# rpp0/gr-lora

Hardware: AMD Instinct MI355X
Metric: IQ Msamples/s demodulated (higher is better)
Workload: dtype f32

## Files before the change

gr_lora_amd/capi.py:

```python
from __future__ import annotations

import ctypes as C
import os
from typing import List, Optional, Sequence, Tuple

import numpy as np

_HERE = os.path.dirname(os.path.abspath(__file__))
LIB_PATH = os.environ.get("LORA_HIP_LIB") or os.path.join(_HERE, "liblora_hip.so")

DEMOD_GRAD, DEMOD_FFT, DEMOD_FFT_COMPAT = 0, 1, 2
FLAG_TRACE = 1
FLAG_PIN_HOST = 2
FLAG_FAST_SYNC = 4
FLAG_NO_DECOUPLED = 8
IQ_CF32, IQ_SC16, IQ_SC8, IQ_CU8 = 0, 1, 2, 3

EXPORTS = [
    "lora_hip_abi_version", "lora_hip_strerror", "lora_hip_last_error", "lora_hip_create", "lora_hip_destroy",
    "lora_hip_get_geometry", "lora_hip_set_sf", "lora_hip_set_samp_rate", "lora_hip_work", "lora_hip_flush",
    "lora_hip_decode_device", "lora_hip_frames_available", "lora_hip_poll_frame", "lora_hip_drain_frames", "lora_hip_drain_slots", "lora_hip_demod_symbols_device", "lora_hip_demod_symbols_ex_device",
    "lora_hip_last_timing", "lora_hip_last_plan", "lora_hip_get_table", "lora_hip_last_payload_pass", "lora_hip_gap_starts_device", "lora_hip_decode_device_begin", "lora_hip_decode_device_end", "lora_hip_decode_device_prepass", "lora_hip_trace", "lora_hip_trace_clear", "lora_hip_check_frame", "lora_hip_estimate_cfo_device", "lora_hip_ref_ifreq_device",
    "lora_hip_set_stream_latency", "lora_hip_stream_info", "lora_hip_walker_kernel_name", "lora_hip_window_stats_device", "lora_hip_detect_preambles_device", "lora_hip_decode_at_headers_device",
    "lora_hip_mux_create", "lora_hip_mux_destroy", "lora_hip_mux_work", "lora_hip_mux_flush", "lora_hip_mux_set_latency", "lora_hip_mux_set_max_ahead", "lora_hip_mux_frames_available",
    "lora_hip_mux_poll_frame", "lora_hip_mux_passes", "lora_hip_mux_last_error",
    "lora_hip_iq_item_bytes", "lora_hip_iq_unpack_device", "lora_hip_work_raw",
]


EXPORTS_CHANNELIZER = [
    "lora_hip_channelizer_create", "lora_hip_channelizer_destroy", "lora_hip_channelizer_last_error", "lora_hip_channelizer_taps",
    "lora_hip_channelizer_output_items", "lora_hip_channelizer_run_device", "lora_hip_channelizer_work", "lora_hip_channelizer_apply_cfo",
    "lora_hip_channelizer_last_kernel_ms", "lora_hip_channelizer_run_device_raw", "lora_hip_channelizer_work_raw",
]


EXPORTS_FILTERBANK = [
# ... 144 lines not shown
    L.lora_hip_get_geometry.argtypes = [vp, C.POINTER(C.c_uint32), C.POINTER(C.c_uint32), C.POINTER(C.c_uint32)]
    L.lora_hip_set_sf.argtypes = [vp, C.c_uint8]
    L.lora_hip_set_samp_rate.argtypes = [vp, C.c_float]
    L.lora_hip_work.argtypes = [vp, vp, C.c_size_t, C.POINTER(C.c_size_t)]
    L.lora_hip_flush.argtypes = [vp]
    L.lora_hip_decode_device.argtypes = [vp, vp, C.c_size_t, vp, vp, C.c_uint32, vp]
    L.lora_hip_frames_available.restype = C.c_size_t
    L.lora_hip_frames_available.argtypes = [vp]
    L.lora_hip_poll_frame.argtypes = [vp, vp, C.c_size_t, C.POINTER(C.c_size_t), C.POINTER(FrameInfo)]
    L.lora_hip_drain_frames.argtypes = [vp, vp, C.c_size_t, C.POINTER(FrameInfo), C.c_size_t, C.POINTER(C.c_size_t)]
    L.lora_hip_drain_slots.argtypes = [vp, vp, C.c_size_t, C.c_size_t, C.POINTER(C.c_size_t)]
    L.lora_hip_demod_symbols_device.argtypes = [vp, vp, C.c_size_t, vp, C.c_size_t, C.c_int, vp, vp]
    L.lora_hip_demod_symbols_ex_device.argtypes = [vp, vp, C.c_size_t, vp, C.c_size_t, C.c_int, vp, vp, vp]
    L.lora_hip_last_timing.argtypes = [vp, C.POINTER(Timing)]
    L.lora_hip_last_plan.argtypes = [vp, C.POINTER(C.c_uint32), C.POINTER(C.c_uint32)]
    L.lora_hip_last_payload_pass.argtypes = [vp, C.POINTER(C.c_uint32), C.POINTER(C.c_uint32), C.POINTER(C.c_uint32), C.POINTER(C.c_uint32), C.POINTER(C.c_uint32), C.POINTER(C.c_float)]
    L.lora_hip_decode_device_begin.argtypes = [vp, vp, C.c_size_t, vp, vp, C.c_uint32, vp, C.c_uint32]
    L.lora_hip_decode_device_end.argtypes = [vp]
    L.lora_hip_decode_device_prepass.argtypes = [vp, vp, C.c_size_t, vp, vp, C.c_uint32, vp, C.c_uint32]
    L.lora_hip_gap_starts_device.argtypes = [vp, vp, C.c_size_t, vp, vp, C.c_uint32, vp, C.c_size_t, vp, vp]
    L.lora_hip_trace.restype = C.c_size_t
    L.lora_hip_trace.argtypes = [vp, C.POINTER(C.POINTER(Step))]
    L.lora_hip_trace_clear.argtypes = [vp]
    L.lora_hip_trace_clear.restype = None
    L.lora_hip_estimate_cfo_device.argtypes = [vp, vp, C.c_size_t, C.POINTER(C.c_int64), C.c_size_t, C.c_int, C.POINTER(C.c_float), vp]
    L.lora_hip_estimate_cfo_device.restype = C.c_int
    L.lora_hip_ref_ifreq_device.argtypes = [vp, vp, C.c_size_t, C.POINTER(C.c_float), C.POINTER(C.c_float), vp]
    L.lora_hip_ref_ifreq_device.restype = C.c_int
    if hasattr(L, "lora_hip_get_table") or not os.environ.get("LORA_HIP_LIB"):
        L.lora_hip_get_table.argtypes = [vp, C.c_int, C.POINTER(C.c_float), C.c_size_t, C.POINTER(C.c_size_t)]
# ... 325 lines not shown
        self._check(self.L.lora_hip_last_plan(self.h, C.byref(b), C.byref(n)))
        return bool(b.value), int(n.value)

    def table(self, which: int) -> np.ndarray:
        n = C.c_size_t()
        self._check(self.L.lora_hip_get_table(self.h, which, None, 0, C.byref(n)))
        out = np.empty(n.value, np.float32)
        self._check(self.L.lora_hip_get_table(self.h, which, out.ctypes.data_as(C.POINTER(C.c_float)), n.value, C.byref(n)))
        return out

    def payload_pass(self):
        a, mv, b, r, c, m = C.c_uint32(0), C.c_uint32(0), C.c_uint32(0), C.c_uint32(0), C.c_uint32(0), C.c_float(0)
        self._check(self.L.lora_hip_last_payload_pass(self.h, C.byref(a), C.byref(mv), C.byref(b), C.byref(r), C.byref(c), C.byref(m)))
        return dict(packets=int(a.value), moved=int(mv.value), rerun=int(b.value), rounds=int(r.value), symbols=int(c.value), ms=float(m.value))

    def trace(self):
        p = C.POINTER(Step)()
        n = self.L.lora_hip_trace(self.h, C.byref(p))
        return [(p[i].state, p[i].pos, p[i].consumed, p[i].bin, p[i].fine, p[i].value, p[i].stream, p[i].cycles) for i in range(n)]

    def trace_clear(self):
        self.L.lora_hip_trace_clear(self.h)


class Mux:

    def __init__(self, n_channels, samp_rate=1e6, bandwidth=125000, sf=7, implicit=False, cr=4, crc=True, reduced_rate=False,
                 disable_drift_correction=False, device=0, demod=DEMOD_FFT_COMPAT, flags=0, segment_symbols=0, batch_items=0):
        self.L = load()
        cfg = Config(struct_size=C.sizeof(Config), samp_rate=float(samp_rate), bandwidth=int(bandwidth), sf=int(sf), implicit=int(bool(implicit)), cr=int(cr),
# ... 366 lines not shown
```

gr_lora_amd/csrc/lora_device.h:

```cpp
#pragma once
#include <stdint.h>

#if !defined(__HIPCC__) && !defined(HIP_INCLUDE_HIP_HIP_RUNTIME_H)
struct float2 { float x, y; };
#endif

namespace lora_hip {

constexpr int kWG = 256;
constexpr int kMaxBinsPerThread = 16;
constexpr int kMaxFrame = 3 + 255 + 2;
constexpr int kMaxCodewords = 640;

enum DecState : int32_t { kDetect = 0, kSync, kFindSfd, kPause, kDecodeHeader, kDecodePayload, kStop };

enum AttemptStatus : uint32_t {
    kAttemptNone = 0,
    kAttemptFrame = 1,
    kAttemptLostSync = 2,
    kAttemptOutOfData = 3,
    kAttemptAtHeader = 4,
    kAttemptAtSfd = 5,
    kAttemptHeaderOnly = 6
};
// ... 73 lines not shown
    int64_t  final_pos;
    uint32_t n_attempts;
    uint32_t final_cr;
    uint32_t npush;
    float    push_tail[4];
    uint32_t stop_reason;
    uint32_t n_steps;
    uint32_t pad;
    uint32_t cyc[6];
    uint32_t rounds[6];
    int64_t  tail_final_pos;
    uint32_t tail_valid, tail_first_rec, tail_n_attempts, tail_final_cr, tail_npush, tail_stop_reason, tail_pad, tail_rsv;
    float    tail_push_tail[4];
    uint32_t ctl[4];
    uint32_t dbg[6];
};

struct StepRec {
    int32_t  state, consumed;
    int64_t  pos;
    int32_t  bin, fine;
    float    value;
    uint32_t stream;
    uint32_t cycles;
    uint32_t pad;
};

struct LaunchCfg {
    const float2 *iq;
    const Job *jobs;
    JobResult *results;
    AttemptRec *recs;
    uint32_t recs_per_job;
    float *scratch;
    StepRec *trace;
    uint32_t trace_cap;
    uint32_t n_jobs;
    uint32_t *balance;
    uint32_t skip_payload;
};
constexpr uint32_t kBalanceCus = 2048;
constexpr uint32_t kBalanceWords = 3u * kBalanceCus;

struct EnvStream {
    uint64_t off;
    uint32_t first_block;
    uint32_t n_blocks;
};
int launch_envelope(const float2 *iq, const EnvStream *streams , uint32_t n_streams, uint32_t sps,
                    float *d_E, unsigned long long *d_bitmap , void *stream);

int launch_walker(const DevParams &p, const LaunchCfg &c, void *stream);
const char *walker_kernel_name(const DevParams &p);
struct DemodAlt { int32_t *shift; uint32_t *bins; int32_t *fine; int64_t max_start; };
// ... 23 lines not shown
bool walker_has_skip_variant(const DevParams &p);
int launch_ref_ifreq(const float2 *x, uint32_t n, float *d_arg, float *d_ifreq, void *stream);
int launch_cfo(const DevParams &p, const float2 *iq, const int64_t *d_offsets, uint32_t n, int mode, float *d_out, void *stream);
bool walker3_covers(uint32_t sf);
uint32_t w3_tw_entries(uint32_t sf);
void build_w3_tables(uint32_t sf, float2 *tw, float2 *ctab );
uint32_t wave_tables_floats(uint32_t sf);
void build_wave_tables(uint32_t sf, const float2 *down, float *out);
uint32_t wave_tables_floats_d(uint32_t sf, uint32_t decim);
void build_wave_tables_d(uint32_t sf, uint32_t decim, const float2 *down, float *out);
uint32_t team_tables_entries(uint32_t sf);
void build_team_tables(uint32_t sf, const float2 *down, double dt, double bandwidth, float2 *out);
uint32_t walker_lds_bytes(const DevParams &p);
uint32_t walker_resident_slots(const DevParams &p);
uint32_t walker_resident_slots_full(const DevParams &p);
const char *walker_kernel_name_for(const DevParams &p, uint32_t n_jobs, bool skip = false);

}
```

gr_lora_amd/csrc/lora_kernels.hip:

```cpp

#include <hip/hip_runtime.h>
#include <math.h>
#include <stdio.h>
#include <atomic>
#include <cstdlib>
#include <stdint.h>
#include <type_traits>

#include "lora_device.h"
#include "whitening_data.inc"

namespace lora_hip {

__constant__ unsigned char c_whiten_cr56[LORA_WHITEN_CR56_LEN];
__constant__ unsigned char c_whiten_cr78[LORA_WHITEN_CR78_LEN];
__constant__ unsigned char c_h84_decode[256];
static std::atomic<bool> g_consts_ready[16];

static unsigned char h_hamming_encode(unsigned v)
{
    const unsigned b0 = v & 1u, b1 = (v >> 1) & 1u, b2 = (v >> 2) & 1u, b3 = (v >> 3) & 1u;
    const unsigned p1 = b1 ^ b2 ^ b3, p2 = b0 ^ b1 ^ b2, p3 = b0 ^ b1 ^ b3, p4 = b0 ^ b2 ^ b3;
    return (unsigned char)(p1 | (b0 << 1) | (b1 << 2) | (b2 << 3) | (p2 << 4) | (b3 << 5) | (p3 << 6) | (p4 << 7));
}
// ... 1053 lines not shown
            cus_dev = dev;
        }
        if (n_jobs <= (uint32_t)cus && !no_wide) {
            const bool grad = p.demod_mode == 0u;
            if (p.sf == 8u && !grad) { k.fn = walker2_kernel_sf8_wide; k.name = "walker2_kernel_sf8_wide"; }
            else if (p.sf == 7u && !grad) { k.fn = walker2_kernel_sf7_wide; k.name = "walker2_kernel_sf7_wide"; }
            else if (p.sf == 7u) { k.fn = walker2_kernel_sf7_grad_wide; k.name = "walker2_kernel_sf7_grad_wide"; }
            else { k.fn = walker2_kernel_sf8_grad_wide; k.name = "walker2_kernel_sf8_grad_wide"; }
        }
    }
    return k;
}

const char *walker_kernel_name_for(const DevParams &p, uint32_t n_jobs, bool skip) { return pick_for_launch(p, n_jobs, skip).name; }

int launch_walker(const DevParams &p, const LaunchCfg &c, void *stream)
{
    if (ensure_constants() != 0) return -1;
    if (c.skip_payload && !walker_has_skip_variant(p)) return -1;
    const WalkerKernel k = pick_for_launch(p, c.n_jobs, c.skip_payload != 0);
    if (k.lds > 64u * 1024u) {
        static thread_local const void *last_fn = nullptr;
        static thread_local uint32_t last_lds = 0;
        static thread_local int last_dev = -1;
        int dev = 0;
        (void)hipGetDevice(&dev);
        if (last_fn != (const void *)k.fn || last_lds < k.lds || last_dev != dev) {
            if (hipFuncSetAttribute((const void *)k.fn, hipFuncAttributeMaxDynamicSharedMemorySize, (int)k.lds) != hipSuccess) return -1;
            last_fn = (const void *)k.fn; last_lds = k.lds; last_dev = dev;
        }
// ... 255 lines not shown
```

gr_lora_amd/csrc/lora_runtime.cpp:

```cpp

#include <hip/hip_runtime.h>

#include <algorithm>
#include <cmath>
#include <cstddef>
#include <cstdarg>
#include <cstdio>
#include <cstdlib>
#include <cstring>
#include <chrono>
#include <deque>
#include <new>
#include <string>
#include <vector>

#include "../../include/lora_hip.h"
#include "lora_device.h"
#include "lora_stitch.hpp"
#include "lora_mux_dev.h"
#include "lora_iq.h"

using namespace lora_hip;

namespace {
// ... 101 lines not shown
    DevBuf<Job> d_jobs;
    DevBuf<JobResult> d_results;
    DevBuf<AttemptRec> d_recs;
    DevBuf<float> d_scratch;
    DevBuf<StepRec> d_trace;
    DevBuf<float2> d_staging;
    DevBuf<int64_t> d_offsets;
    DevBuf<uint32_t> d_bins;
    RunOut run_out[2];
    std::vector<JobResult> h_results;
    std::vector<AttemptRec> h_recs;
    std::vector<StepRec> h_trace;
    hipEvent_t ev0 = nullptr, ev1 = nullptr, ev_done = nullptr;
    hipEvent_t ev_pre0 = nullptr, ev_pre1 = nullptr, ev_dep = nullptr;
    hipStream_t pre_stream = nullptr;
    struct Pending { uint32_t nj = 0, recs_per_job = 0, eager = 0, trace_cap = 0; bool direct = true, open = false; hipStream_t st = nullptr;
                     std::chrono::steady_clock::time_point hp0, hp1; } pending;
    PassCtx pass;
    std::vector<StreamDesc> pass_streams;
    const float2 *pass_iq = nullptr;
    hipStream_t pass_st = nullptr;
    bool pass_open = false, iq_ready = false;
    bool pre_issued = false;
    const float2 *pre_iq = nullptr;
    uint64_t pre_sig = 0;
    uint32_t pre_ns = 0;
    std::chrono::steady_clock::time_point pre_hq0;
    FrameQueue frames;
    PinnedBuf<Job> p_jobs;
    PinnedBuf<JobResult> p_res;
    PinnedBuf<AttemptRec> p_recs;
// ... 9 lines not shown
    ChunkPipe pipe;
    struct HostFeed {
        PinnedBuf<float2> stage[2];
        hipEvent_t stage_ev[2] = {nullptr, nullptr};
        bool stage_busy[2] = {false, false};
        int stage_i = 0;
        DevBuf<uint32_t> d_raw;
        std::vector<std::pair<uintptr_t, uintptr_t>> pinned;
        std::vector<std::pair<uintptr_t, uintptr_t>> refused;
    } feed;
    const char *last_kernel = nullptr;
    uint32_t last_kernel_jobs = 0;
    uint32_t resident_slots = 0;
    uint32_t resident_slots_alt = ~0u;
    uint32_t eager_recs = 4;
    uint32_t last_plan_burst = 0, last_plan_segments = 0;
    int decoupled_policy = -1;
    bool launch_skip = false;
    uint32_t dec_backoff = 0;
    uint32_t last_payload_packets = 0, last_payload_rerun = 0, last_payload_symbols = 0, last_payload_moved = 0, last_payload_rounds = 0;
    float last_payload_ms = 0.0f;
    PinnedBuf<int64_t> p_pay_off;
    PinnedBuf<PayloadDesc> p_pay_desc;
    PinnedBuf<PayloadOut> p_pay_out;
    DevBuf<int32_t> d_fine, d_alt_shift, d_alt_fine;
    DevBuf<uint32_t> d_alt_bins;
    hipStream_t pay_stream = nullptr;
    hipEvent_t ev_pay0 = nullptr, ev_pay1 = nullptr, ev_pay_done = nullptr;
    struct PayState { std::vector<uint32_t> active; size_t used = 0, cap_sym = 0, n_sym = 0; int round = 0; float ms = 0.0f; bool open = false; } pay;
};
// ... 224 lines not shown
    HIP_TRY(h, h->p_recs.reserve((size_t)nj * eager));
    std::memcpy(h->p_jobs.p, jobs.data(), nj * sizeof(Job));
    if (!direct) HIP_TRY(h, hipMemcpyAsync(h->d_jobs.p, h->p_jobs.p, nj * sizeof(Job), hipMemcpyHostToDevice, st));
    LaunchCfg c{};
    c.iq = d_iq; c.recs_per_job = recs_per_job;
    c.jobs = direct ? h->p_jobs.p : h->d_jobs.p; c.results = direct ? h->p_res.p : h->d_results.p; c.recs = direct ? h->p_recs.p : h->d_recs.p;
    c.scratch = need_scratch ? h->d_scratch.p : nullptr;
    c.trace = trace_cap ? h->d_trace.p : nullptr; c.trace_cap = trace_cap; c.n_jobs = nj;
    static const bool no_balance = getenv("LORA_HIP_NO_BALANCE") != nullptr;
    if (!h->d_balance.p && !no_balance) {
        HIP_TRY(h, h->d_balance.reserve(kBalanceWords));
        HIP_TRY(h, hipMemsetAsync(h->d_balance.p, 0, kBalanceWords * sizeof(uint32_t), st));
    }
    c.balance = no_balance ? nullptr : h->d_balance.p;
    c.skip_payload = h->launch_skip ? 1u : 0u;
    HIP_TRY(h, hipEventRecord(h->ev0, st));
    if (nj >= h->last_kernel_jobs) { h->last_kernel = walker_kernel_name_for(h->P, nj, h->launch_skip); h->last_kernel_jobs = nj; }
    if (launch_walker(h->P, c, st) != 0) return fail(h, LORA_HIP_ERR_HIP, "walker launch failed: %s", hipGetErrorString(hipGetLastError()));
    HIP_TRY(h, hipEventRecord(h->ev1, st));
    if (!direct) {
        HIP_TRY(h, hipMemcpyAsync(h->p_res.p, h->d_results.p, nj * sizeof(JobResult), hipMemcpyDeviceToHost, st));
        HIP_TRY(h, hipMemcpy2DAsync(h->p_recs.p, eager * sizeof(AttemptRec), h->d_recs.p, recs_per_job * sizeof(AttemptRec), eager * sizeof(AttemptRec), nj,
                                    hipMemcpyDeviceToHost, st));
    }
    HIP_TRY(h, hipEventRecord(h->ev_done, st));
    h->pending.eager = eager; h->pending.direct = direct; h->pending.open = true;
    h->pending.hp1 = std::chrono::steady_clock::now();
    return LORA_HIP_OK;
}

// ... 61 lines not shown
    }
    if (dbg_stats && h->P.use_fast) {
        double sync_rounds = 0; uint32_t frames = 0, tails = 0, early = 0;
        for (uint32_t j = 0; j < nj; j++) {
            const JobResult &r = out.res[j];
            sync_rounds += r.rounds[1];
            const uint32_t used = std::min(std::min(eager, max_att), r.n_attempts + (r.tail_valid ? r.tail_n_attempts : 0u));
            for (uint32_t a = 0; a < used; a++) {
                const AttemptRec &t = out.recs[(size_t)j * stride + a];
                frames += (a < r.n_attempts && t.status == kAttemptFrame) ? 1u : 0u;
                if (r.tail_valid && a + 1u == r.n_attempts + r.tail_n_attempts && r.tail_pad) { tails++; early += t.status == kAttemptAtSfd ? 1u : 0u; }
            }
        }
        fprintf(stderr, "[lora_hip] acquisitions: %.0f SYNC rounds for %u frames of this launch (%.2f per frame); %u tail probes reached a packet, %u of them stopped behind their first FIND_SFD step\n",
                sync_rounds, frames, frames ? sync_rounds / frames : 0.0, tails, early);
    }
    h->eager_recs = std::min(std::max(max_att, 2u), 8u);
    bool more = false;
    if (max_att > eager) {
        HIP_TRY(h, hipMemcpy2DAsync(out.recs.data() + eager, stride * sizeof(AttemptRec), h->d_recs.p + eager,
                                    recs_per_job * sizeof(AttemptRec), (max_att - eager) * sizeof(AttemptRec), nj, hipMemcpyDeviceToHost, st));
        more = true;
    }
    if (trace_cap) {
        h->h_trace.resize((size_t)nj * trace_cap);
        HIP_TRY(h, hipMemcpyAsync(h->h_trace.data(), h->d_trace.p, (size_t)nj * trace_cap * sizeof(StepRec), hipMemcpyDeviceToHost, st));
        more = true;
    }
    if (more) HIP_TRY(h, hipStreamSynchronize(st));
    float ms = 0.0f;
// ... 1373 lines not shown
    return LORA_HIP_OK;
}

lora_hip_status lora_hip_last_payload_pass(const lora_hip_decoder_t *h, uint32_t *packets, uint32_t *moved, uint32_t *rerun, uint32_t *rounds, uint32_t *symbols, float *ms)
{
    if (!h) return LORA_HIP_ERR_ARG;
    if (packets) *packets = h->last_payload_packets;
    if (moved) *moved = h->last_payload_moved;
    if (rounds) *rounds = h->last_payload_rounds;
    if (rerun) *rerun = h->last_payload_rerun;
    if (symbols) *symbols = h->last_payload_symbols;
    if (ms) *ms = h->last_payload_ms;
    return LORA_HIP_OK;
}

const char *lora_hip_walker_kernel_name(const lora_hip_decoder_t *h) { return h ? (h->last_kernel ? h->last_kernel : walker_kernel_name(h->P)) : ""; }

lora_hip_status lora_hip_last_timing(const lora_hip_decoder_t *h, lora_hip_timing_t *t)
{
    if (!h || !t) return LORA_HIP_ERR_ARG;
    *t = h->timing;
    return LORA_HIP_OK;
}

size_t lora_hip_trace(const lora_hip_decoder_t *h, const lora_hip_step_t **steps)
{
    if (!h || !steps) return 0;
    *steps = h->trace.data();
    return h->trace.size();
}
// ... 8 lines not shown
```

gr_lora_amd/csrc/lora_walker2.inc.hip:

```cpp

constexpr int kW2DetectK = 4;
#ifndef LORA_W2_WAVES_SF7
#define LORA_W2_WAVES_SF7 8
#endif
#ifndef LORA_W2_WAVES_SF8
#define LORA_W2_WAVES_SF8 8
#endif
#ifndef LORA_W2_SFD_K
#define LORA_W2_SFD_K 2
#endif
#ifndef LORA_W2_EU_SF8
#define LORA_W2_EU_SF8 4
#endif
constexpr int kW2MaxWaves = LORA_W2_WAVES_SF7 > LORA_W2_WAVES_SF8 ? LORA_W2_WAVES_SF7 : LORA_W2_WAVES_SF8;

constexpr int kW2SfdK = LORA_W2_SFD_K;

enum W2Mode : int32_t { kPlanExit = 0, kPlanDetect, kPlanSync, kPlanSfd, kPlanPause, kPlanDecode, kPlanFinalize };

struct alignas(16) W2Plan {
    int64_t pos;
    int32_t mode;
    int32_t buf;
    int32_t resolve_prev;
    int32_t n_win;
    int32_t prev_n;
    int32_t zmode;
};

struct alignas(16) W2State {
    int64_t  pos, att_start, att_trig, att_hdr;
// ... 21 lines not shown
    float    specf[kW2MaxWaves][4];
    float    detf[kW2MaxWaves * kW2DetectK][4];
    int32_t  detn[kW2MaxWaves];
    int32_t  speci[2][kW2MaxWaves][4];
    W2Plan   plan[2];
    Shared   sh;
    W2State  st;
    W2Stats  stats;
    int64_t  ph_start;
    uint32_t ph_go, ph_cr, ph_natt, ph_pad;
    uint32_t det_streak;
    uint32_t prio;
    uint32_t words_pk[2];
    strict::Cands sc;
    uint32_t words_pk16[4];
};

struct W2Tabs {
    const float  *v;
    const float  *dd;
    float        *scratch;
};

template <int WAVES>
__device__ __forceinline__ void w2_block_argmax_first(float &v, int &idx, float *red)
{
    const int lane = threadIdx.x & 63, wave = threadIdx.x >> 6;
#pragma unroll
    for (int o = 32; o > 0; o >>= 1) {
        const float ov = __shfl_xor(v, o, 64);
// ... 120 lines not shown
            S.state = kDecodePayload;
        }
        return false;
    }
    if (block_done && !P.implicit) S.payload_symbols -= (int32_t)(4u + S.cr);
    if (S.payload_symbols <= 0) {
        uint32_t n_bytes;
        if (S.cr >= 3u) n_bytes = (uint32_t)ceilf((float)S.n_cw * 4.0f / (4.0f + (float)S.cr));
        else n_bytes = (S.n_cw + 1u) / 2u;
        if (n_bytes > (uint32_t)(kMaxCodewords / 2 + 8)) n_bytes = kMaxCodewords / 2 + 8;
        S.fin_n_bytes = n_bytes;
        S.fin_plen = S.payload_length > 257u ? 257u : S.payload_length;
        return true;
    }
    return false;
}

template <int SF>
__device__ __forceinline__ float4 w2_detect_window(const float2 *p_)
{
    const auto p = (const __attribute__((address_space(1))) v2f *)p_;
    constexpr int SPS = 8 << SF, J = SPS / 64;
    const int lane = threadIdx.x & 63;
    float a0 = 0.f, a1 = 0.f, a2 = 0.f, a3 = 0.f;
    constexpr int B = J < 16 ? J : 16;
#pragma unroll
    for (int jb = 0; jb < J; jb += B) {
        v2f u[B], w[B];
#pragma unroll
        for (int j = 0; j < B; j++) u[j] = p[(jb + j) * 64 + lane];
// ... 312 lines not shown
        default:
            pl.mode = kPlanDecode; pl.n_win = kW2Win;
            if (S.state == kDecodePayload && !P.implicit) {
                const int32_t rem = S.payload_symbols - (int32_t)S.n_words;
                pl.n_win = rem < kW2Win ? (rem > 0 ? rem : 1) : kW2Win;
            }
            break;
        }
    };
    auto plan_from_state = [&](W2Plan &pl) { plan_from(S, pl); };

    W2Tabs T{vl, ddl, W.red};
    uint32_t *bal_mine = nullptr, *bal_other = nullptr;
    uint32_t bal_rem = 0xffffffffu, bal_seen = 0u, bal_slot = 0u;
    if (t0) W.prio = 0u;
    if (t0 && C.balance) {
        const uint32_t hw = __builtin_amdgcn_s_getreg((31 << 11) | 4), xcc = __builtin_amdgcn_s_getreg((31 << 11) | 20);
        const uint32_t cu = ((xcc & 7u) << 8) | ((hw >> 8) & 0xffu);
        bal_slot = atomicAdd(&C.balance[2u * kBalanceCus + cu], 1u) & 1u;
        bal_mine = C.balance + 2u * cu + bal_slot;
        bal_other = C.balance + 2u * cu + (bal_slot ^ 1u);
    }
    for (int phase = 0; phase < 2; phase++) {
    if (t0) {
        S = W2State{};
        S.state = kDetect; S.pos = job.start; S.cr = job.cr_prev; S.has_crc = P.ctor_crc;
        S.phdr[1] = (uint8_t)((P.ctor_cr << 5) | (P.ctor_crc << 4));
        S.att_start = job.start; S.att_trig = -1; S.att_hdr = -1; S.att_cr_prev = job.cr_prev;
        if (job.start_at_header && phase == 0) { S.state = kDecodeHeader; S.in_attempt = 1; S.att_trig = job.start; S.att_hdr = job.start; }
        if (phase == 0) W.stats = W2Stats{};
// ... 23 lines not shown
        if (t0 && bal_mine) {
            W.prio = (bal_rem > bal_seen || (bal_rem == bal_seen && bal_slot != 0u)) ? 1u : 0u;
            const int64_t target = phase == 0 ? job.scan_limit + (job.probe_limit > job.scan_limit ? 12 * (int64_t)sps : 0) : pos + 6 * (int64_t)sps;
            const int64_t left = (target - pos) / (int64_t)sps;
            bal_rem = left < 1 ? 1u : (left > 0x3fffffff ? 0x3fffffffu : (uint32_t)left);
            __hip_atomic_store(bal_mine, bal_rem, __ATOMIC_RELAXED, __HIP_MEMORY_SCOPE_AGENT);
            bal_seen = __hip_atomic_load(bal_other, __ATOMIC_RELAXED, __HIP_MEMORY_SCOPE_AGENT);
        }
        if (!is_ctl) {
            if (W.prio) __builtin_amdgcn_s_setprio(1); else __builtin_amdgcn_s_setprio(0);
        }
        const int64_t wpos = pos + (int64_t)wave * sps;

        if (plan_mode == kPlanDetect) {
            const int kd = plan_n_win;
            if (!is_ctl) {
                const int64_t dpos = pos + (int64_t)wave * kd * sps;
                int nvalid = 0;
                if (dpos + 2 * (int64_t)sps <= n_items) {
                    const int64_t fit = (n_items - dpos) / (int64_t)sps - 1;
                    nvalid = fit < kd ? (int)fit : kd;
                }
                float a[kW2DetectK][4];
                if (nvalid > 0) {
                    if (kd == 1) { const float4 r = w2_detect_window<GSF>(X + dpos); a[0][0] = r.x; a[0][1] = r.y; a[0][2] = r.z; a[0][3] = r.w; }
                    else w2_detect_windows<GSF, kW2DetectK>(X + dpos, nvalid, a);
                }
                if (lane == 0) {
                    W.detn[wave] = nvalid;
                    for (int i = 0; i < kW2DetectK; i++)
                        if (i < nvalid) { float *o = W.detf[wave * kW2DetectK + i]; o[0] = a[i][0]; o[1] = a[i][1]; o[2] = a[i][2]; o[3] = a[i][3]; }
// ... 9 lines not shown
                const bool valid = q < NW && qi < W.detn[qw];
                float autocorr = 0.0f, pushed = 0.0f, e2 = 0.0f;
                if (valid) {
                    const float *o = W.detf[qw * kW2DetectK + qi];
                    const float d0 = o[0], d1 = o[1], e1 = o[2];
                    e2 = o[3];
                    pushed = e1 / (float)sps;
                    const float sq = sqrtf(e1 * e2);
                    autocorr = hypotf(d0 / sq, d1 / sq);
                }
                const unsigned long long vmask = __ballot(valid), tmask = __ballot(valid && autocorr >= 0.90f);
                W.red[q] = pushed; W.red[64 + q] = e2; W.red[128 + q] = autocorr;
                __builtin_amdgcn_wave_barrier();
                if (t0) {
                    W2State L = S;
                    int64_t n_lim = (job.scan_limit - L.pos + (int64_t)sps - 1) / (int64_t)sps;
                    if (n_lim < 1) n_lim = 1;
                    const int n_valid = (~vmask == 0ull) ? 64 : __builtin_ctzll(~vmask);
                    int n_max = n_valid < NW ? n_valid : NW;
                    if ((int64_t)n_max > n_lim) n_max = (int)n_lim;
                    const int qt = tmask ? __builtin_ctzll(tmask) : 64;
                    const bool trig = qt < n_max;
                    const int nd = trig ? qt + 1 : n_max;
                    if (nd > 0) {
                        if (trace) {
                            for (int i = 0; i < nd; i++) {
                                if (L.n_steps + (uint32_t)i < C.trace_cap) {
                                    StepRec &r = trace[L.n_steps + (uint32_t)i];
                                    r.state = kDetect; r.consumed = (trig && i == nd - 1) ? 0 : (int32_t)sps; r.pos = L.pos + (int64_t)i * sps; r.bin = -1; r.fine = 0;
                                    r.value = W.red[128 + i]; r.stream = job.stream_id; r.cycles = (uint32_t)(clock64() - t_start); r.pad = 0;
// ... 152 lines not shown
        }

        if (plan_mode == kPlanFinalize) {
            const uint32_t n_cw = S.n_cw, cr = S.cr, n_bytes = S.fin_n_bytes, plen = S.fin_plen;
            decode_payload_bytes(sh, n_cw, cr, n_bytes);
            AttemptRec &r = recs[S.n_att];
            for (uint32_t i = threadIdx.x; i < plen; i += kW2) r.frame[3u + i] = (i < n_bytes) ? sh.dec[i] : 0;
            __syncthreads();
            if (t0) {
                r.frame[0] = S.phdr[0]; r.frame[1] = S.phdr[1]; r.frame[2] = S.phdr[2];
                r.frame_len = 3u + plen;
                S.frame_ok = 1;
                S.state = kDetect;
                S.n_words = 0; S.n_cw = 0;
                S.fin_pending = 0;
                w2_end_step(S, job, C, recs, trace, S.fin_st, S.fin_consumed, S.fin_bin, S.fin_fine, 0.0f, t_start);
                plan_from_state(next);
            }
            continue;
        }

        int64_t dpos = pos;
        int32_t dn = plan_n_win;
        if (plan_resolve_prev && plan_prev_n > 0) {
            const int rb = plan_buf ^ 1;
            const int32_t s_l = lane < plan_prev_n ? W.speci[rb][lane][0] : -1, f_l = lane < plan_prev_n ? W.speci[rb][lane][1] : 0;
            const unsigned long long moved = __ballot(s_l >= 0 && f_l != 0);
            if (moved) {
                const int wq = __builtin_ctzll(moved);
                const int32_t redo = plan_prev_n - (wq + 1);
// ... 95 lines not shown
            } else {
                plan_from(L, np, zreq);
            }
            const long long tr3 = clock64();
            if (t0) {
                next = np;
                S = L;
                if constexpr (W16) { W.words_pk16[0] = wpk[0]; W.words_pk16[1] = wpk[1]; W.words_pk16[2] = wpk[2]; W.words_pk16[3] = wpk[3]; }
                else { W.words_pk[0] = wpk[0]; W.words_pk[1] = wpk[1]; }
                asm volatile("s_waitcnt lgkmcnt(0)" ::: "memory");
                W.stats.ctl[0] += (uint32_t)((tr1 - tr0) >> 6); W.stats.ctl[1] += (uint32_t)((tr2 - tr1) >> 6); W.stats.ctl[2] += (uint32_t)((tr3 - tr2) >> 6);
                W.stats.ctl[3] += (uint32_t)((clock64() - tr3) >> 6);
                W.stats.cyc[4] += (uint32_t)((clock64() - tr0) >> 6); W.stats.rounds[4]++;
            }
        }
    }

    __syncthreads();
    if (t0) {
        const bool in_attempt = S.in_attempt != 0;
        if (in_attempt && S.n_att < rec_cap) {
            AttemptRec &r = recs[S.n_att];
            r.status = (S.stop_reason == 3) ? kAttemptAtHeader : kAttemptOutOfData;
            r.start_pos = S.att_start; r.trig_pos = S.att_trig; r.hdr_pos = S.att_hdr; r.end_pos = S.pos;
            r.npush = S.npush;
            for (int i = 0; i < 4; i++) r.push_tail[i] = S.push_tail[i];
            r.cr_prev = S.att_cr_prev; r.hdr_ambig = S.att_ambig; r.n_symbols = S.n_sym; r.frame_len = 0; r.n_sfd = 0;
        }
        JobResult &jr = C.results[jid];
        const int64_t e_pos = in_attempt ? S.att_start : S.pos;
// ... 10 lines not shown
            jr.pad = e_pad;
            jr.tail_valid = 0;
            go = job.probe_limit > job.scan_limit && S.stop_reason == 0 && !in_attempt && !trace && e_natt < C.recs_per_job;
            W.ph_go = go ? 1u : 0u; W.ph_start = e_pos; W.ph_cr = S.cr; W.ph_natt = e_natt; W.ph_pad = 0;
        } else {
            jr.tail_valid = 1; jr.tail_first_rec = W.ph_natt;
            jr.tail_final_pos = e_pos; jr.tail_n_attempts = e_natt; jr.tail_final_cr = S.cr; jr.tail_npush = e_npush;
            for (int i = 0; i < 4; i++) jr.tail_push_tail[i] = S.push_tail[i];
            jr.tail_stop_reason = (uint32_t)S.stop_reason; jr.tail_pad = e_pad; jr.tail_rsv = 0;
        }
        if (!go) {
            W2Stats &Q = W.stats;
            if (Q.prev_state >= 0) { Q.cyc[Q.prev_state] += (uint32_t)((clock64() - Q.prev_t) >> 6); Q.rounds[Q.prev_state]++; }
            for (int i = 0; i < 6; i++) { jr.cyc[i] = Q.cyc[i]; jr.rounds[i] = Q.rounds[i]; }
            for (int i = 0; i < 4; i++) jr.ctl[i] = Q.ctl[i];
            jr.dbg[0] = __builtin_amdgcn_s_getreg((31 << 11) | 4); jr.dbg[1] = __builtin_amdgcn_s_getreg((31 << 11) | 20);
            jr.dbg[2] = dbg_t0; jr.dbg[3] = (uint32_t)__builtin_amdgcn_s_memrealtime();
            jr.dbg[4] = dbg_c0; jr.dbg[5] = (uint32_t)(clock64() >> 6);
        }
    }
    if (phase == 1) break;
    __syncthreads();
    if (!W.ph_go) break;
    bal_rem = 0xffffffffu;
    {
        const int64_t st = W.ph_start;
        const uint32_t lo = __builtin_amdgcn_readfirstlane((uint32_t)st), hi = __builtin_amdgcn_readfirstlane((uint32_t)((uint64_t)st >> 32));
        const uint32_t natt = __builtin_amdgcn_readfirstlane(W.ph_natt);
        job.start = (int64_t)(((uint64_t)hi << 32) | lo);
        job.cr_prev = __builtin_amdgcn_readfirstlane(W.ph_cr);
// ... 58 lines not shown
```

include/lora_hip.h:

```cpp
#ifndef LORA_HIP_H
#define LORA_HIP_H

#include <stddef.h>
#include <stdint.h>

#ifdef __cplusplus
extern "C" {
#endif

#define LORA_HIP_ABI_VERSION 4

typedef enum lora_hip_status {
    LORA_HIP_OK = 0,
    LORA_HIP_ERR_BAD_SF = -1,
    LORA_HIP_ERR_BAD_CONFIG = -2,
    LORA_HIP_ERR_NO_DEVICE = -3,
    LORA_HIP_ERR_HIP = -4,
    LORA_HIP_ERR_NOMEM = -5,
    LORA_HIP_ERR_ARG = -6,
    LORA_HIP_ERR_OVERFLOW = -7,
    LORA_HIP_ERR_INTERNAL = -8
} lora_hip_status;

typedef enum lora_hip_iq_format {
// ... 133 lines not shown
                                      size_t max_frames, size_t *n_frames);

lora_hip_status lora_hip_drain_slots(lora_hip_decoder_t *h, uint8_t *slots, size_t slot_bytes, size_t max_slots,
                                     size_t *n_frames);

lora_hip_status lora_hip_demod_symbols_device(lora_hip_decoder_t *h, const void *d_iq, size_t total_items,
                                              const int64_t *offsets, size_t n, int demod,
                                              uint32_t *bins_out, void *hip_stream);

lora_hip_status lora_hip_demod_symbols_ex_device(lora_hip_decoder_t *h, const void *d_iq, size_t total_items,
                                                 const int64_t *offsets, size_t n, int demod,
                                                 uint32_t *bins_out, int32_t *fine_out, void *hip_stream);

lora_hip_status lora_hip_last_timing(const lora_hip_decoder_t *h, lora_hip_timing_t *t);
const char     *lora_hip_walker_kernel_name(const lora_hip_decoder_t *h);
lora_hip_status lora_hip_last_payload_pass(const lora_hip_decoder_t *h, uint32_t *packets, uint32_t *moved, uint32_t *rerun, uint32_t *rounds,
                                           uint32_t *symbols, float *ms);

lora_hip_status lora_hip_last_plan(const lora_hip_decoder_t *h, uint32_t *burst_aware, uint32_t *segments);
lora_hip_status lora_hip_get_table(const lora_hip_decoder_t *h, int which, float *buf, size_t cap_floats, size_t *n_floats);
size_t          lora_hip_trace(const lora_hip_decoder_t *h, const lora_hip_step_t **steps);
void            lora_hip_trace_clear(lora_hip_decoder_t *h);

lora_hip_status lora_hip_estimate_cfo_device(lora_hip_decoder_t *h, const void *d_iq, size_t total_items,
                                             const int64_t *offsets, size_t n, int mode, float *cfo_hz_out,
                                             void *hip_stream);

lora_hip_status lora_hip_ref_ifreq_device(lora_hip_decoder_t *h, const void *d_iq, size_t n_items, float *arg_out, float *ifreq_out,
                                          void *hip_stream);

// ... 42 lines not shown
```

Baseline: 263,900.

## Fuse packet-end payload decode with next DETECT window in SF7 walker

```diff
diff --git a/gr_lora_amd/capi.py b/gr_lora_amd/capi.py
--- a/gr_lora_amd/capi.py
+++ b/gr_lora_amd/capi.py
@@ -20,7 +20,7 @@
     "lora_hip_abi_version", "lora_hip_strerror", "lora_hip_last_error", "lora_hip_create", "lora_hip_destroy",
     "lora_hip_get_geometry", "lora_hip_set_sf", "lora_hip_set_samp_rate", "lora_hip_work", "lora_hip_flush",
     "lora_hip_decode_device", "lora_hip_frames_available", "lora_hip_poll_frame", "lora_hip_drain_frames", "lora_hip_drain_slots", "lora_hip_demod_symbols_device", "lora_hip_demod_symbols_ex_device",
-    "lora_hip_last_timing", "lora_hip_last_plan", "lora_hip_get_table", "lora_hip_last_payload_pass", "lora_hip_gap_starts_device", "lora_hip_decode_device_begin", "lora_hip_decode_device_end", "lora_hip_decode_device_prepass", "lora_hip_trace", "lora_hip_trace_clear", "lora_hip_check_frame", "lora_hip_estimate_cfo_device", "lora_hip_ref_ifreq_device",
+    "lora_hip_last_timing", "lora_hip_last_plan", "lora_hip_get_table", "lora_hip_last_payload_pass", "lora_hip_chain_stats", "lora_hip_gap_starts_device", "lora_hip_decode_device_begin", "lora_hip_decode_device_end", "lora_hip_decode_device_prepass", "lora_hip_trace", "lora_hip_trace_clear", "lora_hip_check_frame", "lora_hip_estimate_cfo_device", "lora_hip_ref_ifreq_device",
     "lora_hip_set_stream_latency", "lora_hip_stream_info", "lora_hip_walker_kernel_name", "lora_hip_window_stats_device", "lora_hip_detect_preambles_device", "lora_hip_decode_at_headers_device",
     "lora_hip_mux_create", "lora_hip_mux_destroy", "lora_hip_mux_work", "lora_hip_mux_flush", "lora_hip_mux_set_latency", "lora_hip_mux_set_max_ahead", "lora_hip_mux_frames_available",
     "lora_hip_mux_poll_frame", "lora_hip_mux_passes", "lora_hip_mux_last_error",
@@ -195,6 +195,8 @@
     L.lora_hip_demod_symbols_ex_device.argtypes = [vp, vp, C.c_size_t, vp, C.c_size_t, C.c_int, vp, vp, vp]
     L.lora_hip_last_timing.argtypes = [vp, C.POINTER(Timing)]
     L.lora_hip_last_plan.argtypes = [vp, C.POINTER(C.c_uint32), C.POINTER(C.c_uint32)]
+    if hasattr(L, "lora_hip_chain_stats") or not os.environ.get("LORA_HIP_LIB"):
+        L.lora_hip_chain_stats.argtypes = [vp, C.POINTER(C.c_uint64)]
     L.lora_hip_last_payload_pass.argtypes = [vp, C.POINTER(C.c_uint32), C.POINTER(C.c_uint32), C.POINTER(C.c_uint32), C.POINTER(C.c_uint32), C.POINTER(C.c_uint32), C.POINTER(C.c_float)]
     L.lora_hip_decode_device_begin.argtypes = [vp, vp, C.c_size_t, vp, vp, C.c_uint32, vp, C.c_uint32]
     L.lora_hip_decode_device_end.argtypes = [vp]
@@ -550,6 +552,11 @@
         self._check(self.L.lora_hip_last_payload_pass(self.h, C.byref(a), C.byref(mv), C.byref(b), C.byref(r), C.byref(c), C.byref(m)))
         return dict(packets=int(a.value), moved=int(mv.value), rerun=int(b.value), rounds=int(r.value), symbols=int(c.value), ms=float(m.value))
 
+    def chain_stats(self):
+        a = (C.c_uint64 * 4)()
+        self._check(self.L.lora_hip_chain_stats(self.h, a))
+        return dict(packet_ends=int(a[2]), fused_ends=int(a[3]))
+
     def trace(self):
         p = C.POINTER(Step)()
         n = self.L.lora_hip_trace(self.h, C.byref(p))
diff --git a/gr_lora_amd/csrc/lora_device.h b/gr_lora_amd/csrc/lora_device.h
--- a/gr_lora_amd/csrc/lora_device.h
+++ b/gr_lora_amd/csrc/lora_device.h
@@ -111,6 +111,7 @@
     float    tail_push_tail[4];
     uint32_t ctl[4];
     uint32_t dbg[6];
+    uint32_t chain[4];
 };
 
 struct StepRec {
@@ -135,6 +136,7 @@
     uint32_t n_jobs;
     uint32_t *balance;
     uint32_t skip_payload;
+    uint32_t no_fuse_end;
 };
 constexpr uint32_t kBalanceCus = 2048;
 constexpr uint32_t kBalanceWords = 3u * kBalanceCus;
@@ -188,6 +190,7 @@
 uint32_t walker_lds_bytes(const DevParams &p);
 uint32_t walker_resident_slots(const DevParams &p);
 uint32_t walker_resident_slots_full(const DevParams &p);
+bool walker_reports_chain(const DevParams &p, bool skip);
 const char *walker_kernel_name_for(const DevParams &p, uint32_t n_jobs, bool skip = false);
 
 }
diff --git a/gr_lora_amd/csrc/lora_kernels.hip b/gr_lora_amd/csrc/lora_kernels.hip
--- a/gr_lora_amd/csrc/lora_kernels.hip
+++ b/gr_lora_amd/csrc/lora_kernels.hip
@@ -1091,6 +1091,15 @@
 
 const char *walker_kernel_name_for(const DevParams &p, uint32_t n_jobs, bool skip) { return pick_for_launch(p, n_jobs, skip).name; }
 
+bool walker_reports_chain(const DevParams &p, bool skip)
+{
+    if (skip || !use_fast_kernel(p)) return false;
+    const bool g = p.demod_mode == 0u;
+    if (p.sf == 7u) return g ? w2_fuse_end<7, true, false, 3>() : w2_fuse_end<7, false, false, 3>();
+    if (p.sf == 8u) return g ? w2_fuse_end<8, true, false, 3>() : w2_fuse_end<8, false, false, 3>();
+    return false;
+}
+
 int launch_walker(const DevParams &p, const LaunchCfg &c, void *stream)
 {
     if (ensure_constants() != 0) return -1;
diff --git a/gr_lora_amd/csrc/lora_runtime.cpp b/gr_lora_amd/csrc/lora_runtime.cpp
--- a/gr_lora_amd/csrc/lora_runtime.cpp
+++ b/gr_lora_amd/csrc/lora_runtime.cpp
@@ -139,7 +139,7 @@
     hipEvent_t ev0 = nullptr, ev1 = nullptr, ev_done = nullptr;
     hipEvent_t ev_pre0 = nullptr, ev_pre1 = nullptr, ev_dep = nullptr;
     hipStream_t pre_stream = nullptr;
-    struct Pending { uint32_t nj = 0, recs_per_job = 0, eager = 0, trace_cap = 0; bool direct = true, open = false; hipStream_t st = nullptr;
+    struct Pending { uint32_t nj = 0, recs_per_job = 0, eager = 0, trace_cap = 0; bool direct = true, open = false, w2 = false; hipStream_t st = nullptr;
                      std::chrono::steady_clock::time_point hp0, hp1; } pending;
     PassCtx pass;
     std::vector<StreamDesc> pass_streams;
@@ -179,6 +179,7 @@
     uint32_t resident_slots = 0;
     uint32_t resident_slots_alt = ~0u;
     uint32_t eager_recs = 4;
+    uint64_t chain[4] = {0, 0, 0, 0};
     uint32_t last_plan_burst = 0, last_plan_segments = 0;
     int decoupled_policy = -1;
     bool launch_skip = false;
@@ -433,6 +434,9 @@
     }
     c.balance = no_balance ? nullptr : h->d_balance.p;
     c.skip_payload = h->launch_skip ? 1u : 0u;
+    static const bool no_fuse_end = getenv("LORA_HIP_NO_FUSE_END") != nullptr;
+    c.no_fuse_end = no_fuse_end ? 1u : 0u;
+    h->pending.w2 = walker_reports_chain(h->P, h->launch_skip);
     HIP_TRY(h, hipEventRecord(h->ev0, st));
     if (nj >= h->last_kernel_jobs) { h->last_kernel = walker_kernel_name_for(h->P, nj, h->launch_skip); h->last_kernel_jobs = nj; }
     if (launch_walker(h->P, c, st) != 0) return fail(h, LORA_HIP_ERR_HIP, "walker launch failed: %s", hipGetErrorString(hipGetLastError()));
@@ -524,6 +528,13 @@
         }
         fprintf(stderr, "[lora_hip] acquisitions: %.0f SYNC rounds for %u frames of this launch (%.2f per frame); %u tail probes reached a packet, %u of them stopped behind their first FIND_SFD step\n",
                 sync_rounds, frames, frames ? sync_rounds / frames : 0.0, tails, early);
+    }
+    if (h->pending.w2) {
+        uint64_t ch[4] = {0, 0, 0, 0};
+        for (uint32_t j = 0; j < nj; j++) for (int i = 0; i < 4; i++) ch[i] += out.res[j].chain[i];
+        for (int i = 0; i < 4; i++) h->chain[i] += ch[i];
+        if (dbg_stats) fprintf(stderr, "[lora_hip] packet ends: %llu finalised by this launch's jobs, %llu of them took the DETECT step behind the packet from the windows evaluated in the packet's last round\n",
+                               (unsigned long long)ch[2], (unsigned long long)ch[3]);
     }
     h->eager_recs = std::min(std::max(max_att, 2u), 8u);
     bool more = false;
@@ -1927,6 +1938,13 @@
     return LORA_HIP_OK;
 }
 
+lora_hip_status lora_hip_chain_stats(const lora_hip_decoder_t *h, uint64_t out[4])
+{
+    if (!h || !out) return LORA_HIP_ERR_ARG;
+    for (int i = 0; i < 4; i++) out[i] = h->chain[i];
+    return LORA_HIP_OK;
+}
+
 const char *lora_hip_walker_kernel_name(const lora_hip_decoder_t *h) { return h ? (h->last_kernel ? h->last_kernel : walker_kernel_name(h->P)) : ""; }
 
 lora_hip_status lora_hip_last_timing(const lora_hip_decoder_t *h, lora_hip_timing_t *t)
diff --git a/gr_lora_amd/csrc/lora_walker2.inc.hip b/gr_lora_amd/csrc/lora_walker2.inc.hip
--- a/gr_lora_amd/csrc/lora_walker2.inc.hip
+++ b/gr_lora_amd/csrc/lora_walker2.inc.hip
@@ -15,6 +15,12 @@
 constexpr int kW2MaxWaves = LORA_W2_WAVES_SF7 > LORA_W2_WAVES_SF8 ? LORA_W2_WAVES_SF7 : LORA_W2_WAVES_SF8;
 
 constexpr int kW2SfdK = LORA_W2_SFD_K;
+
+#ifndef LORA_W2_FUSE_END
+#define LORA_W2_FUSE_END 1
+#endif
+template <int SF, bool GRAD, bool SKIP, int LD> constexpr bool w2_fuse_end() { return LORA_W2_FUSE_END != 0 && SF == 7 && LD == 3 && !SKIP; }
+constexpr int64_t kW2NoDetPos = -0x7fffffffffffffffLL - 1;
 
 enum W2Mode : int32_t { kPlanExit = 0, kPlanDetect, kPlanSync, kPlanSfd, kPlanPause, kPlanDecode, kPlanFinalize };
 
@@ -66,6 +72,9 @@
     uint32_t words_pk[2];
     strict::Cands sc;
     uint32_t words_pk16[4];
+    int64_t  det_pos;
+    uint32_t n_pkt_end, n_fused;
+    uint32_t fuse_pad[2];
 };
 
 struct W2Tabs {
@@ -216,6 +225,29 @@
         return true;
     }
     return false;
+}
+
+__device__ __forceinline__ void w2_wave_lds_sync() { __builtin_amdgcn_wave_barrier(); asm volatile("s_waitcnt lgkmcnt(0)" ::: "memory"); __builtin_amdgcn_wave_barrier(); }
+__device__ __forceinline__ void w2_decode_payload_wave(Shared &sh, uint32_t n_cw, uint32_t cr, uint32_t n_bytes)
+{
+    const uint32_t lane = threadIdx.x & 63u;
+    w2_wave_lds_sync();
+    for (uint32_t i = lane; i < n_cw; i += 64u) {
+        uint8_t w = deshuffle_byte(sh.cw[i]);
+        if (cr <= 2u) w ^= (i < LORA_WHITEN_CR56_LEN) ? c_whiten_cr56[i] : 0;
+        else w ^= (i < LORA_WHITEN_CR78_LEN) ? c_whiten_cr78[i] : 0;
+        sh.cw[i] = w;
+    }
+    w2_wave_lds_sync();
+    for (uint32_t k = lane; k < n_bytes; k += 64u) {
+        const uint8_t c0 = (2u * k < n_cw) ? sh.cw[2u * k] : 0, c1 = (2u * k + 1u < n_cw) ? sh.cw[2u * k + 1u] : 0;
+        uint8_t lo, hi;
+        if (cr >= 3u) { lo = c_h84_decode[c0]; hi = c_h84_decode[c1]; }
+        else if (cr >= 1u) { lo = data_bits(c0); hi = data_bits(c1); }
+        else { lo = 0; hi = 0; }
+        sh.dec[k] = (uint8_t)((hi << 4) | lo);
+    }
+    w2_wave_lds_sync();
 }
 
 template <int SF>
@@ -558,6 +590,8 @@
     uint32_t *bal_mine = nullptr, *bal_other = nullptr;
     uint32_t bal_rem = 0xffffffffu, bal_seen = 0u, bal_slot = 0u;
     if (t0) W.prio = 0u;
+    constexpr bool FUSE = w2_fuse_end<SF, GRAD, SKIP, LD>();
+    if constexpr (FUSE) { if (t0) { W.det_pos = kW2NoDetPos; W.n_pkt_end = 0u; W.n_fused = 0u; } }
     if (t0 && C.balance) {
         const uint32_t hw = __builtin_amdgcn_s_getreg((31 << 11) | 4), xcc = __builtin_amdgcn_s_getreg((31 << 11) | 20);
         const uint32_t cu = ((xcc & 7u) << 8) | ((hw >> 8) & 0xffu);
@@ -611,7 +645,9 @@
 
         if (plan_mode == kPlanDetect) {
             const int kd = plan_n_win;
-            if (!is_ctl) {
+            bool have = false;
+            if constexpr (FUSE) have = kd == 1 && W.det_pos == pos;
+            if (!is_ctl && !have) {
                 const int64_t dpos = pos + (int64_t)wave * kd * sps;
                 int nvalid = 0;
                 if (dpos + 2 * (int64_t)sps <= n_items) {
@@ -651,6 +687,7 @@
                 __builtin_amdgcn_wave_barrier();
                 if (t0) {
                     W2State L = S;
+                    if constexpr (FUSE) { if (have) W.n_fused++; W.det_pos = kW2NoDetPos; }
                     int64_t n_lim = (job.scan_limit - L.pos + (int64_t)sps - 1) / (int64_t)sps;
                     if (n_lim < 1) n_lim = 1;
                     const int n_valid = (~vmask == 0ull) ? 64 : __builtin_ctzll(~vmask);
@@ -833,6 +870,7 @@
                 S.state = kDetect;
                 S.n_words = 0; S.n_cw = 0;
                 S.fin_pending = 0;
+                if constexpr (FUSE) W.n_pkt_end++;
                 w2_end_step(S, job, C, recs, trace, S.fin_st, S.fin_consumed, S.fin_bin, S.fin_fine, 0.0f, t_start);
                 plan_from_state(next);
             }
@@ -958,6 +996,40 @@
                 W.stats.cyc[4] += (uint32_t)((clock64() - tr0) >> 6); W.stats.rounds[4]++;
             }
         }
+        if constexpr (FUSE) {
+            const bool end_round = plan_resolve_prev && dn == 0 && dpos == pos && !plan_z && !P.implicit && !C.no_fuse_end;
+            if (end_round) {
+                if (!is_ctl) {
+                    const bool dv = wpos + 2 * (int64_t)sps <= n_items;
+                    float4 r = make_float4(0.f, 0.f, 0.f, 0.f);
+                    if (dv) r = w2_detect_window<GSF>(X + wpos);
+                    if (lane == 0) {
+                        W.detn[wave] = dv ? 1 : 0;
+                        if (dv) { float *o = W.detf[wave * kW2DetectK]; o[0] = r.x; o[1] = r.y; o[2] = r.z; o[3] = r.w; }
+                    }
+                } else {
+                    w2_wave_lds_sync();
+                    if (__builtin_amdgcn_readfirstlane((int32_t)(S.fin_pending != 0u && !S.done)) != 0) {
+                        const uint32_t n_cw = S.n_cw, cr = S.cr, n_bytes = S.fin_n_bytes, plen = S.fin_plen;
+                        w2_decode_payload_wave(sh, n_cw, cr, n_bytes);
+                        AttemptRec &r = recs[S.n_att];
+                        for (uint32_t i = (uint32_t)lane; i < plen; i += 64u) r.frame[3u + i] = (i < n_bytes) ? sh.dec[i] : 0;
+                        if (t0) {
+                            r.frame[0] = S.phdr[0]; r.frame[1] = S.phdr[1]; r.frame[2] = S.phdr[2];
+                            r.frame_len = 3u + plen;
+                            S.frame_ok = 1;
+                            S.state = kDetect;
+                            S.n_words = 0; S.n_cw = 0;
+                            S.fin_pending = 0;
+                            W.n_pkt_end++;
+                            w2_end_step(S, job, C, recs, trace, S.fin_st, S.fin_consumed, S.fin_bin, S.fin_fine, 0.0f, t_start);
+                            plan_from_state(next);
+                            W.det_pos = pos;
+                        }
+                    }
+                }
+            }
+        }
     }
 
     __syncthreads();
@@ -998,6 +1070,7 @@
             if (Q.prev_state >= 0) { Q.cyc[Q.prev_state] += (uint32_t)((clock64() - Q.prev_t) >> 6); Q.rounds[Q.prev_state]++; }
             for (int i = 0; i < 6; i++) { jr.cyc[i] = Q.cyc[i]; jr.rounds[i] = Q.rounds[i]; }
             for (int i = 0; i < 4; i++) jr.ctl[i] = Q.ctl[i];
+            if constexpr (FUSE) { jr.chain[0] = 0u; jr.chain[1] = 0u; jr.chain[2] = W.n_pkt_end; jr.chain[3] = W.n_fused; }
             jr.dbg[0] = __builtin_amdgcn_s_getreg((31 << 11) | 4); jr.dbg[1] = __builtin_amdgcn_s_getreg((31 << 11) | 20);
             jr.dbg[2] = dbg_t0; jr.dbg[3] = (uint32_t)__builtin_amdgcn_s_memrealtime();
             jr.dbg[4] = dbg_c0; jr.dbg[5] = (uint32_t)(clock64() >> 6);
diff --git a/include/lora_hip.h b/include/lora_hip.h
--- a/include/lora_hip.h
+++ b/include/lora_hip.h
@@ -171,6 +171,7 @@
 
 lora_hip_status lora_hip_last_timing(const lora_hip_decoder_t *h, lora_hip_timing_t *t);
 const char     *lora_hip_walker_kernel_name(const lora_hip_decoder_t *h);
+lora_hip_status lora_hip_chain_stats(const lora_hip_decoder_t *h, uint64_t out[4]);
 lora_hip_status lora_hip_last_payload_pass(const lora_hip_decoder_t *h, uint32_t *packets, uint32_t *moved, uint32_t *rerun, uint32_t *rounds,
                                            uint32_t *symbols, float *ms);
 
```

Result: no change. 263,900 (-0.0%).
